# LambdaLabsML/distributed-training-guide

Hardware: AMD Instinct MI355X
Metric: tokens/sec/GPU for Llama-style causal LM at 1/2/4/8 MI355X; peak HBM per GPU (higher is better)
Workload: dtype bf16; 1 GPU; model=llama-3-8b, global_batch=24, seq_len=1024, parallelism=single

## Files before the change

distributed_training_guide_amd/_hip/attention_bwd.hip:

```cpp
#include "attention_common.h"
#include "launchers.h"

template <int D>
__global__ void __launch_bounds__(256) attn_delta_kernel(
    const short* __restrict__ dout, const short* __restrict__ o,
    float* __restrict__ delta, int B, int S, int Hq) {
  const int grp = threadIdx.x >> 4;
  const int gl = threadIdx.x & 15;
  int64_t nrows = (int64_t)B * S * Hq;
  for (int64_t row = (int64_t)blockIdx.x * 16 + grp; row < nrows;
       row += (int64_t)gridDim.x * 16) {
    const short* dp = dout + row * D;
    const short* op = o + row * D;
    float s = 0.f;
#pragma unroll
    for (int i = gl * 8; i < D; i += 16 * 8) {
      bf16x8 dv = *reinterpret_cast<const bf16x8*>(dp + i);
      bf16x8 ov = *reinterpret_cast<const bf16x8*>(op + i);
#pragma unroll
      for (int j = 0; j < 8; ++j) s += bf2f(dv[j]) * bf2f(ov[j]);
    }
#pragma unroll
    for (int off = 1; off < 16; off <<= 1) s += __shfl_xor(s, off, WAVE);
    if (gl == 0) {
      int h = (int)(row % Hq);
      int64_t bs = row / Hq;
      int sp = (int)(bs % S);
      int b = (int)(bs / S);
      delta[((int64_t)b * Hq + h) * S + sp] = s;
    }
  }
}

template <int D, bool DOC>
__global__ void __launch_bounds__(256, 2) attn_dkdv_kernel(
    const short* __restrict__ dout, const short* __restrict__ q,
    const short* __restrict__ k, const short* __restrict__ v,
    const float* __restrict__ lse, const float* __restrict__ delta,
    short* __restrict__ dk, short* __restrict__ dv, int B, int S, int Hq,
    int Hkv, float scale, const int* __restrict__ doc_end) {
  static_assert(D == 64 || D == 128, "head dim must be 64 or 128");
  __shared__ short q_lds[2][64 * D];
  __shared__ short do_lds[2][64 * D];
  __shared__ __attribute__((aligned(16))) float lse_lds[2][64];
  __shared__ __attribute__((aligned(16))) float del_lds[2][64];

  const int nkt = (S + 63) / 64;
  const int group = Hq / Hkv;

  const GroupBlock gb = xcd_remap(blockIdx.x, B * Hkv, nkt);
  const int b = gb.gid / Hkv;
  const int hkv = gb.gid % Hkv;
  const int kt = gb.within;

  const int tid = threadIdx.x;
  const int wid = tid >> 6;
  const int lane = tid & (WAVE - 1);
  const int l15 = lane & 15;
  const int lg = lane >> 4;

  const int kv0 = kt * 64 + wid * 16;
  constexpr int nd16 = D >> 4, nkc = D >> 5;
  const float c2 = scale * LOG2E;
  const int64_t strideS_q = (int64_t)Hq * D;
  const int64_t strideS_kv = (int64_t)Hkv * D;
  const short* kb = k + ((int64_t)b * S * Hkv + hkv) * D;
  const short* vb = v + ((int64_t)b * S * Hkv + hkv) * D;

  bf16x8 kf[nkc], vf[nkc];
  {
    int key = kv0 + l15;
    int keyc = key < S ? key : S - 1;
    const short* kp = kb + (int64_t)keyc * strideS_kv + lg * 8;
    const short* vp = vb + (int64_t)keyc * strideS_kv + lg * 8;
#pragma unroll
    for (int c = 0; c < nkc; ++c) {
      kf[c] = *reinterpret_cast<const bf16x8*>(kp + c * 32);
      vf[c] = *reinterpret_cast<const bf16x8*>(vp + c * 32);
    }
  }

  f32x4 dkacc[nd16], dvacc[nd16];
#pragma unroll
  for (int i = 0; i < nd16; ++i) {
    dkacc[i] = {0.f, 0.f, 0.f, 0.f};
    dvacc[i] = {0.f, 0.f, 0.f, 0.f};
  }

  const int qstart = kt * 64;
  int dend = S, dend_min = S, qcap = S;
  if (DOC) {
    const int* deb = doc_end + (int64_t)b * S;
    dend = deb[min(kv0 + l15, S - 1)];
    dend_min = deb[min(kv0, S - 1)];
    qcap = min(max(deb[min(qstart + 63, S - 1)], qstart + 1), S);
  }
  const int nqt = (qcap - qstart + 63) / 64;
  const int niter = group * nqt;

  auto stage_qdo = [&](int it, int buf) {
    const int64_t hoff = ((int64_t)b * S * Hq + hkv * group + it / nqt) * D;
    stage_tile_pair<D>(q + hoff, dout + hoff, strideS_q,
                       qstart + (it % nqt) * 64, S, q_lds[buf], do_lds[buf],
                       wid, lane);
  };
  auto stage_lse = [&](int it, int buf) {
    const int hh = hkv * group + it / nqt;
    const int qt = qstart + (it % nqt) * 64;
    if (tid < 64) {
      const float* lseb = lse + ((int64_t)b * Hq + hh) * S;
      int rr = qt + tid < S ? qt + tid : S - 1;
      lse_lds[buf][tid] = lseb[rr] * LOG2E;
    } else if (tid < 128) {
      const float* delb = delta + ((int64_t)b * Hq + hh) * S;
      int rr = qt + tid - 64 < S ? qt + tid - 64 : S - 1;
      del_lds[buf][tid - 64] = delb[rr] * scale;
    }
  };

  stage_qdo(0, 0);
  stage_lse(0, 0);
  __syncthreads();

  for (int it = 0; it < niter; ++it) {
    const int buf = it & 1;
    if (it + 1 < niter) {
      stage_qdo(it + 1, buf ^ 1);
      stage_lse(it + 1, buf ^ 1);
    }

    const int qt = qstart + (it % nqt) * 64;
    const short* ql = q_lds[buf];
    const short* dol = do_lds[buf];

    const int key = kv0 + l15;
    const bool diag = (qt < kt * 64 + 64) || (qt + 63 >= S) ||
                      (DOC && qt + 63 >= dend_min);
    u32x4 pk_p[2], pk_ds[2];
    __builtin_amdgcn_s_setprio(1);
#pragma unroll
    for (int mth = 0; mth < 2; ++mth) {
      const int qra = perm16(2 * mth, l15), qrb = perm16(2 * mth + 1, l15);
      f32x4 sa0 = {0.f, 0.f, 0.f, 0.f}, da0 = {0.f, 0.f, 0.f, 0.f};
      f32x4 sa1 = {0.f, 0.f, 0.f, 0.f}, da1 = {0.f, 0.f, 0.f, 0.f};
#pragma unroll
      for (int c = 0; c < nkc; ++c) {
        bf16x8 qa0 = *reinterpret_cast<const bf16x8*>(
            ql + st_idx(qra, c * 32 + lg * 8));
        bf16x8 qa1 = *reinterpret_cast<const bf16x8*>(
            ql + st_idx(qrb, c * 32 + lg * 8));
        bf16x8 do0 = *reinterpret_cast<const bf16x8*>(
            dol + st_idx(qra, c * 32 + lg * 8));
        bf16x8 do1 = *reinterpret_cast<const bf16x8*>(
            dol + st_idx(qrb, c * 32 + lg * 8));
        sa0 = mfma16(qa0, kf[c], sa0);
        sa1 = mfma16(qa1, kf[c], sa1);
        da0 = mfma16(do0, vf[c], da0);
        da1 = mfma16(do1, vf[c], da1);
      }
#pragma unroll
      for (int half = 0; half < 2; ++half) {
        const int mt = 2 * mth + half;
        const f32x4 sa = half ? sa1 : sa0;
        const f32x4 da = half ? da1 : da0;
        const int qoff = cpos16(mt, lg);
        const f32x4 lse4 =
            *reinterpret_cast<const f32x4*>(&lse_lds[buf][qoff]);
        const f32x4 del4 =
            *reinterpret_cast<const f32x4*>(&del_lds[buf][qoff]);
        float e[4], p[4], ds[4];
#pragma unroll
        for (int r = 0; r < 4; ++r)
          e[r] = __builtin_fmaf(sa[r], c2, -lse4[r]);
        if (diag) {
#pragma unroll
          for (int r = 0; r < 4; ++r) {
            const int qrow = qt + qoff + r;
            if (key > qrow || qrow >= S || key >= S || (DOC && qrow >= dend))
              e[r] = -INFINITY;
          }
        }
#pragma unroll
        for (int r = 0; r < 4; ++r) {
          p[r] = __builtin_amdgcn_exp2f(e[r]);
          ds[r] = p[r] * __builtin_fmaf(da[r], scale, -del4[r]);
        }
        const int kc = mt >> 1, rp = (mt & 1) * 2;
        pk_p[kc][rp + 0] = cvt_pk_bf16(p[0], p[1]);
        pk_p[kc][rp + 1] = cvt_pk_bf16(p[2], p[3]);
        pk_ds[kc][rp + 0] = cvt_pk_bf16(ds[0], ds[1]);
        pk_ds[kc][rp + 1] = cvt_pk_bf16(ds[2], ds[3]);
      }
    }

#pragma unroll
    for (int dt = 0; dt < nd16; ++dt) {
#pragma unroll
      for (int kc = 0; kc < 2; ++kc) {
        bf16x8 dofr = tr16_frag_st(dol, kc * 32 + lg * 8, dt * 16, l15);
        bf16x8 qfr = tr16_frag_st(ql, kc * 32 + lg * 8, dt * 16, l15);
        dvacc[dt] = mfma16(__builtin_bit_cast(bf16x8, pk_p[kc]), dofr,
                           dvacc[dt]);
        dkacc[dt] = mfma16(__builtin_bit_cast(bf16x8, pk_ds[kc]), qfr,
                           dkacc[dt]);
      }
    }
    __builtin_amdgcn_s_setprio(0);
    __syncthreads();
  }

#pragma unroll
  for (int r = 0; r < 4; ++r) {
    int keyw = kv0 + lg * 4 + r;
    if (keyw >= S) continue;
    short* dkp = dk + ((int64_t)b * S * Hkv + (int64_t)keyw * Hkv + hkv) * D;
    short* dvp = dv + ((int64_t)b * S * Hkv + (int64_t)keyw * Hkv + hkv) * D;
#pragma unroll
    for (int dt = 0; dt < nd16; ++dt) {
      dkp[dt * 16 + l15] = f2bf(dkacc[dt][r]);
      dvp[dt * 16 + l15] = f2bf(dvacc[dt][r]);
    }
  }
}

template <int D, bool DOC>
__global__ void __launch_bounds__(256, 2) attn_dq_kernel(
    const short* __restrict__ dout, const short* __restrict__ q,
    const short* __restrict__ k, const short* __restrict__ v,
    const float* __restrict__ lse, const float* __restrict__ delta,
    short* __restrict__ dq, int B, int S, int Hq, int Hkv, float scale,
    const int* __restrict__ doc_start) {
  static_assert(D == 64 || D == 128, "head dim must be 64 or 128");
  __shared__ short k_lds[2][KVBLK * D];
  __shared__ short v_lds[2][KVBLK * D];

  const int ntq = (S + QBLK - 1) / QBLK;
  const int gqa = Hq / Hkv;
  const int bpg = gqa * ntq;

  const GroupBlock gb = xcd_remap(blockIdx.x, B * Hkv, bpg);
  const int b = gb.gid / Hkv;
  const int hkv = gb.gid % Hkv;
  const int h = hkv * gqa + gb.within / ntq;
  const int qtile = gb.within % ntq;

  const int tid = threadIdx.x;
  const int wid = tid >> 6;
  const int lane = tid & (WAVE - 1);
  const int l15 = lane & 15;
  const int lg = lane >> 4;

  const int q0 = qtile * QBLK;
  const int rowb[2] = {qgroup_row(q0, wid, 0), qgroup_row(q0, wid, 1)};
  constexpr int nd16 = D >> 4, nkc = D >> 5;
  const float c2 = scale * LOG2E;
  const int64_t strideS_q = (int64_t)Hq * D;
  const int64_t strideS_kv = (int64_t)Hkv * D;
  const short* qb = q + ((int64_t)b * S * Hq + h) * D;
  const short* dob = dout + ((int64_t)b * S * Hq + h) * D;
  const short* kb = k + ((int64_t)b * S * Hkv + hkv) * D;
  const short* vb = v + ((int64_t)b * S * Hkv + hkv) * D;
  const float* lseb = lse + ((int64_t)b * Hq + h) * S;
  const float* delb = delta + ((int64_t)b * Hq + h) * S;

  bf16x8 qf[2][nkc], dof[2][nkc];
  float lse_r[2], del_r[2];
#pragma unroll
  for (int nq = 0; nq < 2; ++nq) {
    int qrow = rowb[nq] + l15;
    int qrc = qrow < S ? qrow : S - 1;
    const short* qp = qb + (int64_t)qrc * strideS_q + lg * 8;
    const short* dop = dob + (int64_t)qrc * strideS_q + lg * 8;
#pragma unroll
    for (int c = 0; c < nkc; ++c) {
      qf[nq][c] = *reinterpret_cast<const bf16x8*>(qp + c * 32);
      dof[nq][c] = *reinterpret_cast<const bf16x8*>(dop + c * 32);
    }
    lse_r[nq] = lseb[qrc] * LOG2E;
    del_r[nq] = delb[qrc] * scale;
  }

  f32x4 dqacc[nd16][2];
#pragma unroll
  for (int dt = 0; dt < nd16; ++dt)
#pragma unroll
    for (int nq = 0; nq < 2; ++nq) dqacc[dt][nq] = {0.f, 0.f, 0.f, 0.f};

  const int kv_end = min(S, q0 + QBLK);
  const int ntiles = (kv_end + KVBLK - 1) / KVBLK;
  int dstart[2], dsmax[2];
  const int t0 =
      doc_window<DOC>(doc_start, b, S, q0, wid, l15, dstart, dsmax);

  auto stage_kv = [&](int t, int buf) {
    stage_tile_pair<D>(kb, vb, strideS_kv, t * KVBLK, S, k_lds[buf],
                       v_lds[buf], wid, lane);
  };
  stage_kv(t0, 0);
  __syncthreads();

  for (int t = t0; t < ntiles; ++t) {
    const int kv0 = t * KVBLK;
    const int buf = tile_buf(t, t0);
    if (t + 1 < ntiles) stage_kv(t + 1, buf ^ 1);

    {
      const bool smask = (kv_end < kv0 + KVBLK);
      u32x4 pk_ds[2][2];
      const short* kl = k_lds[buf];
      const short* vl = v_lds[buf];
      __builtin_amdgcn_s_setprio(1);
#pragma unroll
      for (int mt = 0; mt < 4; ++mt) {
        const int kr = perm16(mt, l15);
        f32x4 s0 = {0.f, 0.f, 0.f, 0.f}, s1 = {0.f, 0.f, 0.f, 0.f};
        f32x4 d0 = {0.f, 0.f, 0.f, 0.f}, d1 = {0.f, 0.f, 0.f, 0.f};
#pragma unroll
        for (int c = 0; c < nkc; ++c) {
          bf16x8 ka = *reinterpret_cast<const bf16x8*>(
              kl + st_idx(kr, c * 32 + lg * 8));
          bf16x8 va = *reinterpret_cast<const bf16x8*>(
              vl + st_idx(kr, c * 32 + lg * 8));
          s0 = mfma16(ka, qf[0][c], s0);
          d0 = mfma16(va, dof[0][c], d0);
          s1 = mfma16(ka, qf[1][c], s1);
          d1 = mfma16(va, dof[1][c], d1);
        }
        const int koff = cpos16(mt, lg);
        const int kc = mt >> 1, rp = (mt & 1) * 2;
#pragma unroll
        for (int nq = 0; nq < 2; ++nq) {
          const int qrow = rowb[nq] + l15;
          const bool diag = (kv0 + KVBLK - 1 > rowb[nq]) || smask ||
                            (DOC && dsmax[nq] > kv0);
          const f32x4 sv = nq ? s1 : s0;
          const f32x4 dv = nq ? d1 : d0;
          float e[4], ds[4];
#pragma unroll
          for (int r = 0; r < 4; ++r)
            e[r] = __builtin_fmaf(sv[r], c2, -lse_r[nq]);
          if (diag) {
#pragma unroll
            for (int r = 0; r < 4; ++r) {
              const int keyr = kv0 + koff + r;
              if (keyr > qrow || keyr >= S || qrow >= S ||
                  (DOC && keyr < dstart[nq]))
                e[r] = -INFINITY;
            }
          }
#pragma unroll
          for (int r = 0; r < 4; ++r)
            ds[r] = __builtin_amdgcn_exp2f(e[r]) *
                    __builtin_fmaf(dv[r], scale, -del_r[nq]);
          pk_ds[nq][kc][rp + 0] = cvt_pk_bf16(ds[0], ds[1]);
          pk_ds[nq][kc][rp + 1] = cvt_pk_bf16(ds[2], ds[3]);
        }
      }

#pragma unroll
      for (int dt = 0; dt < nd16; ++dt) {
#pragma unroll
        for (int kc = 0; kc < 2; ++kc) {
          bf16x8 kfr = tr16_frag_st(kl, kc * 32 + lg * 8, dt * 16, l15);
          dqacc[dt][0] = mfma16(__builtin_bit_cast(bf16x8, pk_ds[0][kc]),
                                kfr, dqacc[dt][0]);
          dqacc[dt][1] = mfma16(__builtin_bit_cast(bf16x8, pk_ds[1][kc]),
                                kfr, dqacc[dt][1]);
        }
      }
      __builtin_amdgcn_s_setprio(0);
    }
    __syncthreads();
  }

#pragma unroll
  for (int nq = 0; nq < 2; ++nq) {
#pragma unroll
    for (int r = 0; r < 4; ++r) {
      int qrow = rowb[nq] + lg * 4 + r;
      if (qrow >= S) continue;
      short* dqp = dq + ((int64_t)b * S * Hq + (int64_t)qrow * Hq + h) * D;
#pragma unroll
      for (int dt = 0; dt < nd16; ++dt) {
        dqp[dt * 16 + l15] = f2bf(dqacc[dt][nq][r]);
      }
    }
  }
}

namespace {
template <int D, bool DOC>
void bwd_launch(const short* dout, const short* q, const short* k,
                const short* v, const short* o, const float* lse,
                float* delta, short* dq, short* dk, short* dv,
                const int* doc_start, const int* doc_end, int B, int S,
                int Hq, int Hkv, float scale, hipStream_t stream) {
  int64_t nrows = (int64_t)B * S * Hq;
  int64_t dwant = (nrows + 15) / 16;
  int dgrid = (int)(dwant < 2048 ? (dwant < 1 ? 1 : dwant) : 2048);
  hipLaunchKernelGGL(attn_delta_kernel<D>, dim3(dgrid), dim3(256), 0, stream,
                     dout, o, delta, B, S, Hq);
  int nkt = (S + 63) / 64;
  hipLaunchKernelGGL((attn_dkdv_kernel<D, DOC>),
                     dim3((uint32_t)((int64_t)B * Hkv * nkt)), dim3(256), 0,
                     stream, dout, q, k, v, lse, delta, dk, dv, B, S, Hq, Hkv,
                     scale, doc_end);
  int ntq = (S + QBLK - 1) / QBLK;
  hipLaunchKernelGGL((attn_dq_kernel<D, DOC>),
                     dim3((uint32_t)((int64_t)B * Hq * ntq)), dim3(256), 0,
                     stream, dout, q, k, v, lse, delta, dq, B, S, Hq, Hkv,
                     scale, doc_start);
}
}

extern "C" void attn_bwd_launch(const void* dout, const void* q, const void* k,
                                const void* v, const void* o, const float* lse,
                                float* delta, void* dq, void* dk, void* dv,
                                const int* doc_start, const int* doc_end,
                                int B, int S, int Hq, int Hkv, int D,
                                float scale, hipStream_t stream) {
  const bool doc = doc_start != nullptr;
  auto fn = doc ? (D == 64 ? bwd_launch<64, true> : bwd_launch<128, true>)
                : (D == 64 ? bwd_launch<64, false> : bwd_launch<128, false>);
  fn((const short*)dout, (const short*)q, (const short*)k, (const short*)v,
     (const short*)o, lse, delta, (short*)dq, (short*)dk, (short*)dv,
     doc_start, doc_end, B, S, Hq, Hkv, scale, stream);
}
```

distributed_training_guide_amd/_hip/attention_common.h:

```cpp
#pragma once
#include "common.h"

using bf16x8 = s16x8;

constexpr int QBLK = 128;
constexpr int KVBLK = 64;
#define LOG2E 1.4426950408889634f

__device__ __forceinline__ f32x4 mfma16(bf16x8 a, bf16x8 b, f32x4 c) {
  return __builtin_amdgcn_mfma_f32_16x16x32_bf16(a, b, c, 0, 0, 0);
}

template <int D>
__device__ __forceinline__ void stage_tile_pair(
    const short* ga, const short* gb, int64_t stride, int row0, int S,
    short* la, short* lb, int wid, int lane) {
  constexpr int ncw = D >> 5;
#pragma unroll
  for (int i = 0; i < ncw; ++i) {
    const int ch = wid * ncw + i;
    int row = row0 + (ch & 1) * 32 + (lane >> 1);
    if (row >= S) row = S - 1;
    const int64_t goff =
        (int64_t)row * stride + (ch >> 1) * 16 + (lane & 1) * 8;
    __builtin_amdgcn_global_load_lds(
        (const __attribute__((address_space(1))) unsigned int*)(ga + goff),
        (LDS_AS unsigned int*)(la + ch * 512), 16, 0, 0);
    __builtin_amdgcn_global_load_lds(
        (const __attribute__((address_space(1))) unsigned int*)(gb + goff),
        (LDS_AS unsigned int*)(lb + ch * 512), 16, 0, 0);
  }
}

struct GroupBlock {
  int gid;
  int within;
};
__device__ __forceinline__ GroupBlock xcd_remap(int bid, int ngroups,
                                                int bpg) {
  if ((ngroups & 7) == 0)
    return {(bid >> 3) / bpg * 8 + (bid & 7), (bid >> 3) % bpg};
  return {bid / bpg, bid % bpg};
}

__device__ __forceinline__ int qgroup_row(int q0, int wid, int nq) {
  return q0 + nq * 64 + wid * 16;
}

template <bool DOC>
__device__ __forceinline__ int doc_window(const int* doc_start, int b, int S,
                                          int q0, int wid, int l15,
                                          int (&dstart)[2], int (&dsmax)[2]) {
  dstart[0] = dstart[1] = dsmax[0] = dsmax[1] = 0;
  if (!DOC) return 0;
  const int* dsb = doc_start + (int64_t)b * S;
#pragma unroll
  for (int nq = 0; nq < 2; ++nq) {
    dstart[nq] = dsb[min(qgroup_row(q0, wid, nq) + l15, S - 1)];
    dsmax[nq] = dsb[min(qgroup_row(q0, wid, nq) + 15, S - 1)];
  }
  return min(max(dsb[q0], 0), q0) / KVBLK;
}

__device__ __forceinline__ int tile_buf(int t, int t0) { return (t - t0) & 1; }
```

distributed_training_guide_amd/_hip/attention_fwd.hip:

```cpp
#include "attention_common.h"
#include "launchers.h"

template <int D, bool DOC>
__global__ void __launch_bounds__(256, 2) attn_fwd_kernel(
    const short* __restrict__ q, const short* __restrict__ k,
    const short* __restrict__ v, short* __restrict__ o,
    float* __restrict__ lse_out, int B, int S, int Hq, int Hkv, float scale,
    const int* __restrict__ doc_start) {
  static_assert(D == 64 || D == 128, "head dim must be 64 or 128");
  __shared__ short k_lds[2][KVBLK * D];
  __shared__ short v_lds[2][KVBLK * D];

  const int ntq = (S + QBLK - 1) / QBLK;
  const int gqa = Hq / Hkv;
  const int bpg = gqa * ntq;

  const GroupBlock gb = xcd_remap(blockIdx.x, B * Hkv, bpg);
  const int b = gb.gid / Hkv;
  const int hkv = gb.gid % Hkv;
  const int h = hkv * gqa + gb.within / ntq;
  const int qtile = gb.within % ntq;

  const int tid = threadIdx.x;
  const int wid = tid >> 6;
  const int lane = tid & (WAVE - 1);
  const int l15 = lane & 15;
  const int lg = lane >> 4;

  const int q0 = qtile * QBLK;
  const int rowb[2] = {qgroup_row(q0, wid, 0), qgroup_row(q0, wid, 1)};
  constexpr int nd16 = D >> 4;
  constexpr int nkc = D >> 5;
  const int64_t strideS_q = (int64_t)Hq * D;
  const int64_t strideS_kv = (int64_t)Hkv * D;
  const short* qb = q + ((int64_t)b * S * Hq + h) * D;
  const short* kb = k + ((int64_t)b * S * Hkv + hkv) * D;
  const short* vb = v + ((int64_t)b * S * Hkv + hkv) * D;

  bf16x8 qf[2][nkc];
#pragma unroll
  for (int nq = 0; nq < 2; ++nq) {
    int qrow = rowb[nq] + l15;
    if (qrow >= S) qrow = S - 1;
    const short* qp = qb + (int64_t)qrow * strideS_q + lg * 8;
#pragma unroll
    for (int kc = 0; kc < nkc; ++kc)
      qf[nq][kc] = *reinterpret_cast<const bf16x8*>(qp + kc * 32);
  }

  int kperm[4], ckey[4];
#pragma unroll
  for (int mt = 0; mt < 4; ++mt) {
    kperm[mt] = perm16(mt, l15);
    ckey[mt] = cpos16(mt, lg);
  }

  f32x4 oacc[nd16][2];
#pragma unroll
  for (int dt = 0; dt < nd16; ++dt)
#pragma unroll
    for (int nq = 0; nq < 2; ++nq) oacc[dt][nq] = {0.f, 0.f, 0.f, 0.f};
  float mrow[2] = {-INFINITY, -INFINITY};
  float mcrow[2] = {-INFINITY, -INFINITY};
  float lrow[2] = {0.f, 0.f};

  const int kv_end = min(S, q0 + QBLK);
  const int ntiles = (kv_end + KVBLK - 1) / KVBLK;
  const float c = scale * LOG2E;
  int dstart[2], dsmax[2];
  const int t0 =
      doc_window<DOC>(doc_start, b, S, q0, wid, l15, dstart, dsmax);

  auto stage_kv = [&](int t, int buf) {
    stage_tile_pair<D>(kb, vb, strideS_kv, t * KVBLK, S, k_lds[buf],
                       v_lds[buf], wid, lane);
  };
  stage_kv(t0, 0);
  __syncthreads();

  for (int t = t0; t < ntiles; ++t) {
    const int kv0 = t * KVBLK;
    const int buf = tile_buf(t, t0);
    if (t + 1 < ntiles) stage_kv(t + 1, buf ^ 1);


    const short* kl = k_lds[buf];
    f32x4 sfrag[4][2];
    __builtin_amdgcn_s_setprio(1);
#pragma unroll
    for (int mth = 0; mth < 2; ++mth) {
      const int kra = kperm[2 * mth], krb = kperm[2 * mth + 1];
      f32x4 a0 = {0.f, 0.f, 0.f, 0.f}, a1 = {0.f, 0.f, 0.f, 0.f};
      f32x4 b0 = {0.f, 0.f, 0.f, 0.f}, b1 = {0.f, 0.f, 0.f, 0.f};
#pragma unroll
      for (int kc = 0; kc < nkc; ++kc) {
        bf16x8 kfa = *reinterpret_cast<const bf16x8*>(
            kl + st_idx(kra, kc * 32 + lg * 8));
        bf16x8 kfb = *reinterpret_cast<const bf16x8*>(
            kl + st_idx(krb, kc * 32 + lg * 8));
        a0 = mfma16(kfa, qf[0][kc], a0);
        b0 = mfma16(kfb, qf[0][kc], b0);
        a1 = mfma16(kfa, qf[1][kc], a1);
        b1 = mfma16(kfb, qf[1][kc], b1);
      }
      sfrag[2 * mth][0] = a0;
      sfrag[2 * mth][1] = a1;
      sfrag[2 * mth + 1][0] = b0;
      sfrag[2 * mth + 1][1] = b1;
    }
    __builtin_amdgcn_s_setprio(0);

    u32x4 pk[2][2];
    float alpha[2];
#pragma unroll
    for (int nq = 0; nq < 2; ++nq) {
      const int qrow = rowb[nq] + l15;
      const bool need_mask = (kv0 + KVBLK - 1) > rowb[nq] ||
                             kv_end < kv0 + KVBLK ||
                             (DOC && dsmax[nq] > kv0);
      if (need_mask) {
#pragma unroll
        for (int mt = 0; mt < 4; ++mt)
#pragma unroll
          for (int r = 0; r < 4; ++r) {
            int key = kv0 + ckey[mt] + r;
            if (key > qrow || key >= S || (DOC && key < dstart[nq]))
              sfrag[mt][nq][r] = -INFINITY;
          }
      }
      float tmax = -INFINITY;
#pragma unroll
      for (int mt = 0; mt < 4; ++mt) {
        f32x4 s = sfrag[mt][nq];
        tmax = fmaxf(tmax, fmaxf(fmaxf(s[0], s[1]), fmaxf(s[2], s[3])));
      }
      tmax = fmaxf(tmax, __shfl_xor(tmax, 16, WAVE));
      tmax = fmaxf(tmax, __shfl_xor(tmax, 32, WAVE));
      const float mnew = fmaxf(mrow[nq], tmax);
      const float mcn = mnew * c;
      const float mc = (mnew == -INFINITY) ? 0.0f : mcn;
      alpha[nq] = __builtin_amdgcn_exp2f(mcrow[nq] - mc);
      mrow[nq] = mnew;
      mcrow[nq] = mcn;
      float psum = 0.f;
#pragma unroll
      for (int mt = 0; mt < 4; ++mt) {
        f32x4 s = sfrag[mt][nq];
        f32x4 p;
#pragma unroll
        for (int r = 0; r < 4; ++r) {
          p[r] = __builtin_amdgcn_exp2f(__builtin_fmaf(s[r], c, -mc));
          psum += p[r];
        }
        pk[nq][mt >> 1][(mt & 1) * 2 + 0] = cvt_pk_bf16(p[0], p[1]);
        pk[nq][mt >> 1][(mt & 1) * 2 + 1] = cvt_pk_bf16(p[2], p[3]);
      }
      psum += __shfl_xor(psum, 16, WAVE);
      psum += __shfl_xor(psum, 32, WAVE);
      lrow[nq] = lrow[nq] * alpha[nq] + psum;
    }

    const short* vt = v_lds[buf];
    __builtin_amdgcn_s_setprio(1);
#pragma unroll
    for (int dt = 0; dt < nd16; ++dt) {
      bf16x8 va[2];
#pragma unroll
      for (int kc = 0; kc < 2; ++kc)
        va[kc] = tr16_frag_st(vt, kc * 32 + lg * 8, dt * 16, l15);
#pragma unroll
      for (int nq = 0; nq < 2; ++nq) {
        f32x4 acc = oacc[dt][nq];
#pragma unroll
        for (int r = 0; r < 4; ++r) acc[r] *= alpha[nq];
        acc = mfma16(va[0], __builtin_bit_cast(bf16x8, pk[nq][0]), acc);
        acc = mfma16(va[1], __builtin_bit_cast(bf16x8, pk[nq][1]), acc);
        oacc[dt][nq] = acc;
      }
    }
    __builtin_amdgcn_s_setprio(0);
    __syncthreads();
  }

#pragma unroll
  for (int nq = 0; nq < 2; ++nq) {
    const int qrow = rowb[nq] + l15;
    if (qrow >= S) continue;
    const float invl = (lrow[nq] > 0.f) ? 1.0f / lrow[nq] : 0.0f;
    short* op = o + ((int64_t)b * S * Hq + (int64_t)qrow * Hq + h) * D;
#pragma unroll
    for (int dt = 0; dt < nd16; ++dt) {
      s16x4 outv;
#pragma unroll
      for (int r = 0; r < 4; ++r) outv[r] = f2bf(oacc[dt][nq][r] * invl);
      *reinterpret_cast<s16x4*>(op + dt * 16 + lg * 4) = outv;
    }
    if (lg == 0)
      lse_out[((int64_t)b * Hq + h) * S + qrow] =
          mrow[nq] * scale + __logf(fmaxf(lrow[nq], 1e-30f));
  }
}

extern "C" void attn_fwd_launch(const void* q, const void* k, const void* v,
                                void* o, float* lse, const int* doc_start,
                                int B, int S, int Hq, int Hkv, int D,
                                float scale, hipStream_t stream) {
  int ntiles = (S + QBLK - 1) / QBLK;
  int64_t grid = (int64_t)B * Hq * ntiles;
  auto kern = doc_start
                  ? (D == 64 ? attn_fwd_kernel<64, true>
                             : attn_fwd_kernel<128, true>)
                  : (D == 64 ? attn_fwd_kernel<64, false>
                             : attn_fwd_kernel<128, false>);
  hipLaunchKernelGGL(kern, dim3((uint32_t)grid), dim3(256), 0, stream,
                     (const short*)q, (const short*)k, (const short*)v,
                     (short*)o, lse, B, S, Hq, Hkv, scale, doc_start);
}
```

Measured before the change: 24280 tokens/s.

## Unroll attention double-buffer loops by two with separate static LDS buffers

Restructures the forward, dkdv and dq attention kernels so the double-buffered loop is unrolled by two, with each half using its own named LDS arrays instead of an index computed from the iteration. Buffer addresses become compile-time constants, and transposed LDS reads use a precomputed per-lane offset, which should cut address arithmetic. In the dkdv kernel the lse/delta global loads for the next tile are issued early and stored to LDS only after compute, so their latency is hidden. This trades larger code and possible register pressure for fewer index calculations and better overlap, and it applies only to head dim 128 where gated.

```diff
diff --git a/distributed_training_guide_amd/_hip/attention_bwd.hip b/distributed_training_guide_amd/_hip/attention_bwd.hip
--- a/distributed_training_guide_amd/_hip/attention_bwd.hip
+++ b/distributed_training_guide_amd/_hip/attention_bwd.hip
@@ -40,10 +40,7 @@
     short* __restrict__ dk, short* __restrict__ dv, int B, int S, int Hq,
     int Hkv, float scale, const int* __restrict__ doc_end) {
   static_assert(D == 64 || D == 128, "head dim must be 64 or 128");
-  __shared__ short q_lds[2][64 * D];
-  __shared__ short do_lds[2][64 * D];
-  __shared__ __attribute__((aligned(16))) float lse_lds[2][64];
-  __shared__ __attribute__((aligned(16))) float del_lds[2][64];
+  constexpr bool PIPE = D == 128;
 
   const int nkt = (S + 63) / 64;
   const int group = Hq / Hkv;
@@ -98,40 +95,49 @@
   const int nqt = (qcap - qstart + 63) / 64;
   const int niter = group * nqt;
 
-  auto stage_qdo = [&](int it, int buf) {
+  auto stage_qdo = [&](int it, short* qn, short* don)
+                       __attribute__((always_inline)) {
     const int64_t hoff = ((int64_t)b * S * Hq + hkv * group + it / nqt) * D;
     stage_tile_pair<D>(q + hoff, dout + hoff, strideS_q,
-                       qstart + (it % nqt) * 64, S, q_lds[buf], do_lds[buf],
-                       wid, lane);
+                       qstart + (it % nqt) * 64, S, qn, don, wid, lane);
   };
-  auto stage_lse = [&](int it, int buf) {
+  auto load_lse = [&](int it) __attribute__((always_inline)) {
     const int hh = hkv * group + it / nqt;
     const int qt = qstart + (it % nqt) * 64;
+    float x = 0.f;
     if (tid < 64) {
       const float* lseb = lse + ((int64_t)b * Hq + hh) * S;
       int rr = qt + tid < S ? qt + tid : S - 1;
-      lse_lds[buf][tid] = lseb[rr] * LOG2E;
+      x = lseb[rr];
     } else if (tid < 128) {
       const float* delb = delta + ((int64_t)b * Hq + hh) * S;
       int rr = qt + tid - 64 < S ? qt + tid - 64 : S - 1;
-      del_lds[buf][tid - 64] = delb[rr] * scale;
-    }
+      x = delb[rr];
+    }
+    return x;
   };
-
-  stage_qdo(0, 0);
-  stage_lse(0, 0);
-  __syncthreads();
-
-  for (int it = 0; it < niter; ++it) {
-    const int buf = it & 1;
-    if (it + 1 < niter) {
-      stage_qdo(it + 1, buf ^ 1);
-      stage_lse(it + 1, buf ^ 1);
+  auto store_lse = [&](float x, float* lsen, float* deln)
+                       __attribute__((always_inline)) {
+    if (tid < 64) {
+      lsen[tid] = x * LOG2E;
+    } else if (tid < 128) {
+      deln[tid - 64] = x * scale;
+    }
+  };
+
+  auto tile = [&](int it, const short* ql, const short* dol,
+                  const float* lsel, const float* dell, short* qn,
+                  short* don, float* lsen, float* deln)
+                  __attribute__((always_inline)) {
+    const bool more = it + 1 < niter;
+    float xnext = 0.f;
+    if (more) {
+      if constexpr (PIPE) xnext = load_lse(it + 1);
+      stage_qdo(it + 1, qn, don);
+      if constexpr (!PIPE) store_lse(load_lse(it + 1), lsen, deln);
     }
 
     const int qt = qstart + (it % nqt) * 64;
-    const short* ql = q_lds[buf];
-    const short* dol = do_lds[buf];
 
     const int key = kv0 + l15;
     const bool diag = (qt < kt * 64 + 64) || (qt + 63 >= S) ||
@@ -165,9 +171,9 @@
         const f32x4 da = half ? da1 : da0;
         const int qoff = cpos16(mt, lg);
         const f32x4 lse4 =
-            *reinterpret_cast<const f32x4*>(&lse_lds[buf][qoff]);
+            *reinterpret_cast<const f32x4*>(&lsel[qoff]);
         const f32x4 del4 =
-            *reinterpret_cast<const f32x4*>(&del_lds[buf][qoff]);
+            *reinterpret_cast<const f32x4*>(&dell[qoff]);
         float e[4], p[4], ds[4];
 #pragma unroll
         for (int r = 0; r < 4; ++r)
@@ -206,7 +212,46 @@
       }
     }
     __builtin_amdgcn_s_setprio(0);
+    if constexpr (PIPE) {
+      if (more) store_lse(xnext, lsen, deln);
+    }
     __syncthreads();
+  };
+
+  if constexpr (PIPE) {
+    __shared__ short q_lds0[64 * D];
+    __shared__ short q_lds1[64 * D];
+    __shared__ short do_lds0[64 * D];
+    __shared__ short do_lds1[64 * D];
+    __shared__ __attribute__((aligned(16))) float lse_lds0[64];
+    __shared__ __attribute__((aligned(16))) float lse_lds1[64];
+    __shared__ __attribute__((aligned(16))) float del_lds0[64];
+    __shared__ __attribute__((aligned(16))) float del_lds1[64];
+    stage_qdo(0, q_lds0, do_lds0);
+    store_lse(load_lse(0), lse_lds0, del_lds0);
+    __syncthreads();
+    for (int it = 0; it < niter; it += 2) {
+      tile(it, q_lds0, do_lds0, lse_lds0, del_lds0, q_lds1, do_lds1,
+           lse_lds1, del_lds1);
+      if (it + 1 >= niter) break;
+      __builtin_amdgcn_sched_barrier(0);
+      tile(it + 1, q_lds1, do_lds1, lse_lds1, del_lds1, q_lds0, do_lds0,
+           lse_lds0, del_lds0);
+    }
+  } else {
+    __shared__ short q_lds[2][64 * D];
+    __shared__ short do_lds[2][64 * D];
+    __shared__ __attribute__((aligned(16))) float lse_lds[2][64];
+    __shared__ __attribute__((aligned(16))) float del_lds[2][64];
+    stage_qdo(0, q_lds[0], do_lds[0]);
+    store_lse(load_lse(0), lse_lds[0], del_lds[0]);
+    __syncthreads();
+    for (int it = 0; it < niter; ++it) {
+      const int buf = it & 1;
+      tile(it, q_lds[buf], do_lds[buf], lse_lds[buf], del_lds[buf],
+           q_lds[buf ^ 1], do_lds[buf ^ 1], lse_lds[buf ^ 1],
+           del_lds[buf ^ 1]);
+    }
   }
 
 #pragma unroll
@@ -231,8 +276,10 @@
     short* __restrict__ dq, int B, int S, int Hq, int Hkv, float scale,
     const int* __restrict__ doc_start) {
   static_assert(D == 64 || D == 128, "head dim must be 64 or 128");
-  __shared__ short k_lds[2][KVBLK * D];
-  __shared__ short v_lds[2][KVBLK * D];
+  __shared__ short k_lds0[KVBLK * D];
+  __shared__ short k_lds1[KVBLK * D];
+  __shared__ short v_lds0[KVBLK * D];
+  __shared__ short v_lds1[KVBLK * D];
 
   const int ntq = (S + QBLK - 1) / QBLK;
   const int gqa = Hq / Hkv;
@@ -291,24 +338,18 @@
   int dstart[2], dsmax[2];
   const int t0 =
       doc_window<DOC>(doc_start, b, S, q0, wid, l15, dstart, dsmax);
-
-  auto stage_kv = [&](int t, int buf) {
-    stage_tile_pair<D>(kb, vb, strideS_kv, t * KVBLK, S, k_lds[buf],
-                       v_lds[buf], wid, lane);
-  };
-  stage_kv(t0, 0);
-  __syncthreads();
-
-  for (int t = t0; t < ntiles; ++t) {
+  const int troff = tr16_lane_off(lg, l15);
+
+  auto tile = [&](int t, const short* kl, const short* vl, short* kn,
+                  short* vn) __attribute__((always_inline)) {
     const int kv0 = t * KVBLK;
-    const int buf = tile_buf(t, t0);
-    if (t + 1 < ntiles) stage_kv(t + 1, buf ^ 1);
+    if (t + 1 < ntiles)
+      stage_tile_pair<D>(kb, vb, strideS_kv, (t + 1) * KVBLK, S, kn, vn, wid,
+                         lane);
 
     {
       const bool smask = (kv_end < kv0 + KVBLK);
       u32x4 pk_ds[2][2];
-      const short* kl = k_lds[buf];
-      const short* vl = v_lds[buf];
       __builtin_amdgcn_s_setprio(1);
 #pragma unroll
       for (int mt = 0; mt < 4; ++mt) {
@@ -361,7 +402,7 @@
       for (int dt = 0; dt < nd16; ++dt) {
 #pragma unroll
         for (int kc = 0; kc < 2; ++kc) {
-          bf16x8 kfr = tr16_frag_st(kl, kc * 32 + lg * 8, dt * 16, l15);
+          bf16x8 kfr = tr16_frag_at(kl + troff, kc, dt);
           dqacc[dt][0] = mfma16(__builtin_bit_cast(bf16x8, pk_ds[0][kc]),
                                 kfr, dqacc[dt][0]);
           dqacc[dt][1] = mfma16(__builtin_bit_cast(bf16x8, pk_ds[1][kc]),
@@ -371,6 +412,16 @@
       __builtin_amdgcn_s_setprio(0);
     }
     __syncthreads();
+  };
+
+  stage_tile_pair<D>(kb, vb, strideS_kv, t0 * KVBLK, S, k_lds0, v_lds0, wid,
+                     lane);
+  __syncthreads();
+  for (int t = t0; t < ntiles; t += 2) {
+    tile(t, k_lds0, v_lds0, k_lds1, v_lds1);
+    if (t + 1 >= ntiles) break;
+    __builtin_amdgcn_sched_barrier(0);
+    tile(t + 1, k_lds1, v_lds1, k_lds0, v_lds0);
   }
 
 #pragma unroll
diff --git a/distributed_training_guide_amd/_hip/attention_common.h b/distributed_training_guide_amd/_hip/attention_common.h
--- a/distributed_training_guide_amd/_hip/attention_common.h
+++ b/distributed_training_guide_amd/_hip/attention_common.h
@@ -32,6 +32,25 @@
   }
 }
 
+__device__ __forceinline__ int tr16_lane_off(int lg, int l15) {
+  return st_idx(lg * 8 + (l15 >> 2), (l15 & 3) * 4);
+}
+__device__ __forceinline__ bf16x8 tr16_frag_at(const short* lane_base, int kc,
+                                               int dt) {
+  const short* p = lane_base + kc * 512 + dt * 1024;
+  s16x4tr lo =
+      __builtin_amdgcn_ds_read_tr16_b64_v4i16((LDS_AS s16x4tr*)p);
+  s16x4tr hi =
+      __builtin_amdgcn_ds_read_tr16_b64_v4i16((LDS_AS s16x4tr*)(p + 64));
+  bf16x8 out;
+#pragma unroll
+  for (int j = 0; j < 4; ++j) {
+    out[j] = lo[j];
+    out[4 + j] = hi[j];
+  }
+  return out;
+}
+
 struct GroupBlock {
   int gid;
   int within;
diff --git a/distributed_training_guide_amd/_hip/attention_fwd.hip b/distributed_training_guide_amd/_hip/attention_fwd.hip
--- a/distributed_training_guide_amd/_hip/attention_fwd.hip
+++ b/distributed_training_guide_amd/_hip/attention_fwd.hip
@@ -8,8 +8,7 @@
     float* __restrict__ lse_out, int B, int S, int Hq, int Hkv, float scale,
     const int* __restrict__ doc_start) {
   static_assert(D == 64 || D == 128, "head dim must be 64 or 128");
-  __shared__ short k_lds[2][KVBLK * D];
-  __shared__ short v_lds[2][KVBLK * D];
+  constexpr bool PIPE = D == 128;
 
   const int ntq = (S + QBLK - 1) / QBLK;
   const int gqa = Hq / Hkv;
@@ -54,6 +53,7 @@
     kperm[mt] = perm16(mt, l15);
     ckey[mt] = cpos16(mt, lg);
   }
+  const int troff = tr16_lane_off(lg, l15);
 
   f32x4 oacc[nd16][2];
 #pragma unroll
@@ -71,20 +71,14 @@
   const int t0 =
       doc_window<DOC>(doc_start, b, S, q0, wid, l15, dstart, dsmax);
 
-  auto stage_kv = [&](int t, int buf) {
-    stage_tile_pair<D>(kb, vb, strideS_kv, t * KVBLK, S, k_lds[buf],
-                       v_lds[buf], wid, lane);
-  };
-  stage_kv(t0, 0);
-  __syncthreads();
-
-  for (int t = t0; t < ntiles; ++t) {
+  auto tile = [&](int t, const short* kl, const short* vt, short* kn,
+                  short* vn) __attribute__((always_inline)) {
     const int kv0 = t * KVBLK;
-    const int buf = tile_buf(t, t0);
-    if (t + 1 < ntiles) stage_kv(t + 1, buf ^ 1);
-
-
-    const short* kl = k_lds[buf];
+    if (t + 1 < ntiles)
+      stage_tile_pair<D>(kb, vb, strideS_kv, (t + 1) * KVBLK, S, kn, vn, wid,
+                         lane);
+
+
     f32x4 sfrag[4][2];
     __builtin_amdgcn_s_setprio(1);
 #pragma unroll
@@ -160,14 +154,14 @@
       lrow[nq] = lrow[nq] * alpha[nq] + psum;
     }
 
-    const short* vt = v_lds[buf];
     __builtin_amdgcn_s_setprio(1);
 #pragma unroll
     for (int dt = 0; dt < nd16; ++dt) {
       bf16x8 va[2];
 #pragma unroll
       for (int kc = 0; kc < 2; ++kc)
-        va[kc] = tr16_frag_st(vt, kc * 32 + lg * 8, dt * 16, l15);
+        va[kc] = PIPE ? tr16_frag_at(vt + troff, kc, dt)
+                      : tr16_frag_st(vt, kc * 32 + lg * 8, dt * 16, l15);
 #pragma unroll
       for (int nq = 0; nq < 2; ++nq) {
         f32x4 acc = oacc[dt][nq];
@@ -180,6 +174,32 @@
     }
     __builtin_amdgcn_s_setprio(0);
     __syncthreads();
+  };
+
+  if constexpr (PIPE) {
+    __shared__ short k_lds0[KVBLK * D];
+    __shared__ short k_lds1[KVBLK * D];
+    __shared__ short v_lds0[KVBLK * D];
+    __shared__ short v_lds1[KVBLK * D];
+    stage_tile_pair<D>(kb, vb, strideS_kv, t0 * KVBLK, S, k_lds0, v_lds0,
+                       wid, lane);
+    __syncthreads();
+    for (int t = t0; t < ntiles; t += 2) {
+      tile(t, k_lds0, v_lds0, k_lds1, v_lds1);
+      if (t + 1 >= ntiles) break;
+      __builtin_amdgcn_sched_barrier(0);
+      tile(t + 1, k_lds1, v_lds1, k_lds0, v_lds0);
+    }
+  } else {
+    __shared__ short k_lds[2][KVBLK * D];
+    __shared__ short v_lds[2][KVBLK * D];
+    stage_tile_pair<D>(kb, vb, strideS_kv, t0 * KVBLK, S, k_lds[0], v_lds[0],
+                       wid, lane);
+    __syncthreads();
+    for (int t = t0; t < ntiles; ++t) {
+      const int buf = tile_buf(t, t0);
+      tile(t, k_lds[buf], v_lds[buf], k_lds[buf ^ 1], v_lds[buf ^ 1]);
+    }
   }
 
 #pragma unroll
```

Result: no change. 24390 tokens/s, median of 2 (+0.5%).
